# MMintLab/gelslim_depth

Measured on AMD Instinct MI355X. Metric: train frames/sec (320x427) at batch 32, higher is better.
Workload: dtype f32

## Files before the change

gelslim_depth_amd/csrc/gsd_convT.hip:

```cpp
#include "gsd_common.h"

namespace {

enum : int { CT_FWD = 1, CT_DGRAD = 2 };

struct ConvTParams {
  SrcD src;
  DstD dst;
  const float* wt;
  const float* bias;
  int K, M, Mpad, nchunks, mblocks;
  int N, H, W;
  int tiles_flat;
};

template <int MODE, int WM, int WN>
__global__ __launch_bounds__(256) void convT_kernel(const ConvTParams P) {
  constexpr int MT = 4, NT = 4;
  constexpr int BM = WM * 64, BN = WN * 64;
  constexpr int KSTEPS = 4;
  constexpr int WROWS = KSTEPS * 4;
  constexpr int WS = BM + 16;
  constexpr int PS = BN + 16;
  constexpr int W4 = WROWS * BM / 4;
// ... 171 lines not shown
      }
  }
}

struct ConvTFwdParams {
  SrcD src;
  DstD dst;
  const float* wt;
  const float* bias;
  int K, Kpad, M, nchunks, mblocks;
  int N, H, W, tiles_flat;
};

__device__ __attribute__((aligned(16))) const float gsd_zero16_ct[4] = {0.f, 0.f, 0.f, 0.f};

template <bool X4>
__global__ __launch_bounds__(256, 2) void convT_fwd_dma_kernel(const ConvTFwdParams P) {
  constexpr int BM = 128, BN = 128, KC = 32, MT = 4, NT = 4;
  constexpr int WIMG = KC * BM, XIMG = KC * BN, BUF = WIMG + XIMG;
  extern __shared__ __attribute__((aligned(16))) float smem[];
  const int tid = threadIdx.x, lane = tid & 63;
  const int wave = __builtin_amdgcn_readfirstlane(tid >> 6);
  const int wm = wave >> 1, wn = wave & 1;
  const int j = lane >> 4, l16 = lane & 15;

  const int lid = xcd_swizzle(blockIdx.x, gridDim.x);
  const int mb = lid % P.mblocks;
  const int pt = lid / P.mblocks;
  const int m0 = mb * BM;
  const long long q0 = (long long)pt * BN;
  const int HW = P.H * P.W;
  const long long QT = (long long)P.N * HW;

  float* sAff = smem + 2 * BUF;
  for (int c = tid; c < P.Kpad; c += 256) {
    float sc = 1.f, sh = 0.f;
    if (c < P.K && P.src.scale != nullptr) {
      sc = P.src.scale[c];
      sh = P.src.shift[c];
    }
    sAff[c] = sc;
    sAff[P.Kpad + c] = sh;
  }
  const float lo = P.src.relu ? 0.f : -__builtin_inff();

  const float* const wsrc = P.wt + (size_t)mb * P.Kpad * BM + lane * 4;
  const int xrow = X4 ? (lane >> 5) : 0;
  const int xpx = X4 ? (lane & 31) * 4 : lane;
  long long xo[X4 ? 1 : 2];
  bool xok[X4 ? 1 : 2];
#pragma unroll
  for (int i = 0; i < (X4 ? 1 : 2); ++i) {
    const long long q = q0 + xpx + 64 * i;
    xok[i] = q < QT;
    const int nn = xok[i] ? (int)(q / HW) : 0;
    xo[i] = (long long)nn * P.src.ns + (xok[i] ? (q - (long long)nn * HW) : 0);
  }
  auto fill = [&](int chunk, int buf) {
    float* Wb = smem + buf * BUF;
    float* Xb = Wb + WIMG;
    const float* wc = wsrc + (size_t)chunk * WIMG;
#pragma unroll
    for (int i = 0; i < 4; ++i) __builtin_amdgcn_global_load_lds(wc + (wave + 4 * i) * 256, Wb + (wave + 4 * i) * 256, 16, 0, 0);
    const int k0 = chunk * KC;
    if constexpr (X4) {
#pragma unroll
      for (int i = 0; i < 4; ++i) {
        const int r = 2 * (wave + 4 * i) + xrow;
        const float* g = (xok[0] && k0 + r < P.K) ? P.src.p + xo[0] + (long long)(k0 + r) * P.src.cs : &gsd_zero16_ct[0];
        __builtin_amdgcn_global_load_lds(g, Xb + (wave + 4 * i) * 256, 16, 0, 0);
      }
    } else {
#pragma unroll
      for (int i = 0; i < 16; ++i) {
        const int u = wave + 4 * i;
        const int r = u >> 1, hf = u & 1;
        const float* g = (xok[hf] && k0 + r < P.K) ? P.src.p + xo[hf] + (long long)(k0 + r) * P.src.cs : &gsd_zero16_ct[0];
        __builtin_amdgcn_global_load_lds(g, Xb + u * 64, 4, 0, 0);
      }
    }
  };

  f32x4 acc[MT][NT];
#pragma unroll
  for (int m = 0; m < MT; ++m)
#pragma unroll
    for (int t = 0; t < NT; ++t) acc[m][t] = f32x4{0.f, 0.f, 0.f, 0.f};

  const int a_off = j * BM + wm * 64 + l16 * 4;
  const int b_off = WIMG + j * BN + wn * 64 + l16 * 4;
  fill(0, 0);
  for (int chunk = 0; chunk < P.nchunks; ++chunk) {
    const int cur = chunk & 1;
    gsd_dma_barrier();
    if (chunk + 1 < P.nchunks) fill(chunk + 1, cur ^ 1);
    const float* Sb = smem + cur * BUF;
    const float* aff = sAff + chunk * KC + j;
    f32x4 av[2], bv[2];
    float sc[2], sh[2];
    av[0] = *reinterpret_cast<const f32x4*>(&Sb[a_off]);
    bv[0] = *reinterpret_cast<const f32x4*>(&Sb[b_off]);
    sc[0] = aff[0];
    sh[0] = aff[P.Kpad];
#pragma unroll
    for (int s = 0; s < KC / 4; ++s) {
      const int c = s & 1;
      if (s + 1 < KC / 4) {
        av[c ^ 1] = *reinterpret_cast<const f32x4*>(&Sb[a_off + (s + 1) * 4 * BM]);
        bv[c ^ 1] = *reinterpret_cast<const f32x4*>(&Sb[b_off + (s + 1) * 4 * BN]);
        sc[c ^ 1] = aff[(s + 1) * 4];
        sh[c ^ 1] = aff[P.Kpad + (s + 1) * 4];
      }
      float b[NT];
#pragma unroll
      for (int t = 0; t < NT; ++t) b[t] = fmaxf(fmaf(bv[c][t], sc[c], sh[c]), lo);
#pragma unroll
      for (int m = 0; m < MT; ++m)
#pragma unroll
        for (int t = 0; t < NT; ++t) acc[m][t] = mfma16(av[c][m], b[t], acc[m][t]);
    }
  }

  typedef float f32x4u __attribute__((ext_vector_type(4), aligned(4)));
  const DstD& D = P.dst;
  const long long qa = q0 + wn * 64 + l16 * 4;
  if (qa < QT) {
    const int na = (int)(qa / HW);
    const int pa = (int)(qa - (long long)na * HW);
    const int ha = pa / P.W, wa = pa - ha * P.W;
    const bool one_row = wa + 3 < P.W;
    if (one_row && qa + 3 < QT) {
      float* const o = D.p + (long long)na * D.ns + (long long)(2 * ha) * D.ws + 2 * wa;
#pragma unroll
      for (int m = 0; m < MT; ++m) {
        const int co = (m0 + wm * 64 + m * 16 + j * 4) >> 2;
        if (co < D.C) {
          const float bz = P.bias != nullptr ? P.bias[co] : 0.f;
          float* const oc = o + (long long)co * D.cs;
          *reinterpret_cast<f32x4u*>(oc) = f32x4{acc[m][0][0] + bz, acc[m][0][1] + bz, acc[m][1][0] + bz, acc[m][1][1] + bz};
          *reinterpret_cast<f32x4u*>(oc + 4) = f32x4{acc[m][2][0] + bz, acc[m][2][1] + bz, acc[m][3][0] + bz, acc[m][3][1] + bz};
          *reinterpret_cast<f32x4u*>(oc + D.ws) = f32x4{acc[m][0][2] + bz, acc[m][0][3] + bz, acc[m][1][2] + bz, acc[m][1][3] + bz};
          *reinterpret_cast<f32x4u*>(oc + D.ws + 4) = f32x4{acc[m][2][2] + bz, acc[m][2][3] + bz, acc[m][3][2] + bz, acc[m][3][3] + bz};
        }
      }
    } else {
#pragma unroll
      for (int t = 0; t < NT; ++t) {
        const long long q = qa + t;
        if (q >= QT) continue;
        const int nn = (int)(q / HW);
        const int p = (int)(q - (long long)nn * HW);
        const int h = p / P.W, w = p - h * P.W;
        float* const o = D.p + (long long)nn * D.ns + (long long)(2 * h) * D.ws + 2 * w;
#pragma unroll
        for (int m = 0; m < MT; ++m) {
          const int co = (m0 + wm * 64 + m * 16 + j * 4) >> 2;
          if (co < D.C) {
            const float bz = P.bias != nullptr ? P.bias[co] : 0.f;
            float* const oc = o + (long long)co * D.cs;
            *reinterpret_cast<float2*>(oc) = make_float2(acc[m][t][0] + bz, acc[m][t][1] + bz);
            *reinterpret_cast<float2*>(oc + D.ws) = make_float2(acc[m][t][2] + bz, acc[m][t][3] + bz);
          }
        }
      }
    }
  }
}

struct ConvTDgParams {
  SrcD src;
  DstD dst;
  const float* wt;
  int K, Kpad, M, nchunks, mblocks;
  int N, H, W, Wv, tiles_flat;
  const float* bw_raw;
  const float* bw_scale;
  const float* bw_shift;
  const float* bw_mean;
  const float* bw_invstd;
  float* partials;
  int Mpad;
};

template <bool BW>
__global__ __launch_bounds__(256, 2) void convT_dgrad_dma_kernel(const ConvTDgParams P) {
  constexpr int BM = 128, BN = 128, KC = 32, MT = 4, NT = 4;
  constexpr int WIMG = KC * BM, XIMG = (KC / 2) * (2 * BN), BUF = WIMG + XIMG;
  extern __shared__ __attribute__((aligned(16))) float smem[];
  const int tid = threadIdx.x, lane = tid & 63;
  const int wave = __builtin_amdgcn_readfirstlane(tid >> 6);
  const int wm = wave >> 1, wn = wave & 1;
  const int j = lane >> 4, l16 = lane & 15;

  const int lid = xcd_swizzle(blockIdx.x, gridDim.x);
  const int mb = lid % P.mblocks;
  const int pt = lid / P.mblocks;
  const int m0 = mb * BM;
  const long long q0 = (long long)pt * BN;
  const int HWv = P.H * P.Wv;
  const long long QT = (long long)P.N * HWv;

  const float* const wsrc = P.wt + (size_t)mb * P.Kpad * BM + lane * 4;
  const int pi = lane ^ ((lane >> 4) & 1);
  long long xo = 0;
  bool xok;
  {
    const long long q = q0 + 2 * pi;
    xok = q < QT;
    const int nn = xok ? (int)(q / HWv) : 0;
    const int rem = xok ? (int)(q - (long long)nn * HWv) : 0;
    const int h = rem / P.Wv, w = rem - h * P.Wv;
    xo = (long long)nn * P.src.ns + (long long)(2 * h) * P.src.ws + 2 * w;
  }
  auto fill = [&](int chunk, int buf) {
    float* Wb = smem + buf * BUF;
    float* Xb = Wb + WIMG;
    const float* wc = wsrc + (size_t)chunk * WIMG;
#pragma unroll
    for (int i = 0; i < 4; ++i) __builtin_amdgcn_global_load_lds(wc + (wave + 4 * i) * 256, Wb + (wave + 4 * i) * 256, 16, 0, 0);
#pragma unroll
    for (int i = 0; i < 4; ++i) {
      const int r = wave + 4 * i;
      const int co = chunk * 8 + (r >> 1);
      const float* g = (xok && co < P.src.C) ? P.src.p + xo + (long long)co * P.src.cs + (long long)(r & 1) * P.src.ws
                                              : &gsd_zero16_ct[0];
      __builtin_amdgcn_global_load_lds(g, Xb + r * 256, 16, 0, 0);
    }
  };

  f32x4 acc[MT][NT];
#pragma unroll
  for (int m = 0; m < MT; ++m)
#pragma unroll
    for (int t = 0; t < NT; ++t) acc[m][t] = f32x4{0.f, 0.f, 0.f, 0.f};

  const int a_off = (2 * j) * BM + wm * 64 + l16 * 4;
  const int lp = 2 * (wn * 16 + l16);
  const int b_off0 = WIMG + j * 256 + 4 * (lp ^ ((lp >> 4) & 1));
  const int b_off1 = WIMG + j * 256 + 4 * ((lp + 1) ^ (((lp + 1) >> 4) & 1));
  fill(0, 0);
  for (int chunk = 0; chunk < P.nchunks; ++chunk) {
    const int cur = chunk & 1;
    gsd_dma_barrier();
    if (chunk + 1 < P.nchunks) fill(chunk + 1, cur ^ 1);
    const float* Sb = smem + cur * BUF;
    f32x4 av[2], x0[2], x1[2];
    av[0] = *reinterpret_cast<const f32x4*>(&Sb[a_off]);
    x0[0] = *reinterpret_cast<const f32x4*>(&Sb[b_off0]);
    x1[0] = *reinterpret_cast<const f32x4*>(&Sb[b_off1]);
#pragma unroll
    for (int s = 0; s < KC / 4; ++s) {
      const int p = s >> 1, kw = s & 1, c = s & 1, pc = p & 1;
      if (s + 1 < KC / 4) {
        av[c ^ 1] = *reinterpret_cast<const f32x4*>(&Sb[a_off + ((s + 1) >> 1) * 8 * BM + ((s + 1) & 1) * BM]);
        if (kw == 1) {
          x0[pc ^ 1] = *reinterpret_cast<const f32x4*>(&Sb[b_off0 + (p + 1) * 4 * 256]);
          x1[pc ^ 1] = *reinterpret_cast<const f32x4*>(&Sb[b_off1 + (p + 1) * 4 * 256]);
        }
      }
      const float b[NT] = {x0[pc][kw], x0[pc][2 + kw], x1[pc][kw], x1[pc][2 + kw]};
#pragma unroll
      for (int m = 0; m < MT; ++m)
#pragma unroll
        for (int t = 0; t < NT; ++t) acc[m][t] = mfma16(av[c][m], b[t], acc[m][t]);
    }
  }

  typedef float f32x4u __attribute__((ext_vector_type(4), aligned(4)));
  const DstD& D = P.dst;
  const long long qa = q0 + wn * 64 + l16 * 4;
  if constexpr (BW) {
    __syncthreads();
    float* sBw = smem;
    if (tid < BM) {
      const int c = m0 + tid < D.C ? m0 + tid : 0;
      sBw[tid] = P.bw_scale[c];
      sBw[BM + tid] = P.bw_shift[c];
      sBw[2 * BM + tid] = P.bw_mean[c];
      sBw[3 * BM + tid] = P.bw_invstd[c];
    }
    __syncthreads();
    long long off[NT];
    bool ok[NT];
#pragma unroll
    for (int t = 0; t < NT; ++t) {
      const long long q = qa + t;
      ok[t] = q < QT;
      const int nn = ok[t] ? (int)(q / HWv) : 0;
      const int r = ok[t] ? (int)(q - (long long)nn * HWv) : 0;
      const int h = r / P.Wv, w = r - h * P.Wv;
      ok[t] = ok[t] && w < P.W;
      off[t] = (long long)nn * D.ns + (long long)h * D.ws + w;
    }
    const bool row4 = ok[0] && ok[3] && off[3] == off[0] + 3;
    float* const prow = P.partials + (size_t)(pt * 2 + wn) * (2 * P.Mpad);
#pragma unroll
    for (int m = 0; m < MT; ++m)
#pragma unroll
      for (int reg = 0; reg < 4; ++reg) {
        const int cl = wm * 64 + m * 16 + j * 4 + reg, ci = m0 + cl;
        const bool c_ok = ci < D.C;
        const long long cp = (long long)(c_ok ? ci : 0) * D.cs;
        const float bsc = sBw[cl], bsh = sBw[BM + cl], bmu = sBw[2 * BM + cl], bis = sBw[3 * BM + cl];
        float x[NT], dz[NT];
        if (row4) {
          const f32x4 tv = *reinterpret_cast<const f32x4u*>(P.bw_raw + cp + off[0]);
          x[0] = tv[0], x[1] = tv[1], x[2] = tv[2], x[3] = tv[3];
        } else {
#pragma unroll
          for (int t = 0; t < NT; ++t) x[t] = ok[t] ? P.bw_raw[cp + off[t]] : 0.f;
        }
        float s1 = 0.f, s2 = 0.f;
#pragma unroll
        for (int t = 0; t < NT; ++t) {
          dz[t] = (c_ok && ok[t] && fmaf(x[t], bsc, bsh) > 0.f) ? acc[m][t][reg] : 0.f;
          s1 += dz[t];
          s2 = fmaf(dz[t], (x[t] - bmu) * bis, s2);
        }
        if (c_ok) {
          if (row4) {
            *reinterpret_cast<f32x4u*>(D.p + cp + off[0]) = f32x4{dz[0], dz[1], dz[2], dz[3]};
          } else {
#pragma unroll
            for (int t = 0; t < NT; ++t)
              if (ok[t]) D.p[cp + off[t]] = dz[t];
          }
        }
        s1 = reduce16_to_lane15(s1);
        s2 = reduce16_to_lane15(s2);
        if (l16 == 15 && ci < P.Mpad) {
          prow[ci] = s1;
          prow[P.Mpad + ci] = s2;
        }
      }
    return;
  }
  if (qa < QT) {
    const int na = (int)(qa / HWv);
    const int ra = (int)(qa - (long long)na * HWv);
    const int ha = ra / P.Wv, wa = ra - ha * P.Wv;
    if (wa + 3 < P.W) {
      float* const o = D.p + (long long)na * D.ns + (long long)ha * D.ws + wa;
#pragma unroll
      for (int m = 0; m < MT; ++m)
#pragma unroll
        for (int reg = 0; reg < 4; ++reg) {
          const int ci = m0 + wm * 64 + m * 16 + j * 4 + reg;
          if (ci < D.C)
            *reinterpret_cast<f32x4u*>(o + (long long)ci * D.cs) = f32x4{acc[m][0][reg], acc[m][1][reg], acc[m][2][reg], acc[m][3][reg]};
// ... 6 lines not shown
        const int nn = (int)(q / HWv);
        const int r = (int)(q - (long long)nn * HWv);
        const int h = r / P.Wv, w = r - h * P.Wv;
        if (w >= P.W) continue;
        float* const o = D.p + (long long)nn * D.ns + (long long)h * D.ws + w;
#pragma unroll
        for (int m = 0; m < MT; ++m)
#pragma unroll
          for (int reg = 0; reg < 4; ++reg) {
            const int ci = m0 + wm * 64 + m * 16 + j * 4 + reg;
            if (ci < D.C) o[(long long)ci * D.cs] = acc[m][t][reg];
          }
      }
    }
  }
}

template <int MODE, int WM, int WN>
int launch(const ConvTParams& P, int grid, size_t lds, hipStream_t st, const char* what) {
  hipLaunchKernelGGL((convT_kernel<MODE, WM, WN>), dim3(grid), dim3(256), lds, st, P);
  GSD_LAUNCH_CHECK(what);
  return GSD_OK;
}

template <int MODE>
int run(ConvTParams& P, hipStream_t st, const char* what) {
  const bool wide = P.M <= 64;
  const int BM = wide ? 64 : 128, BN = wide ? 256 : 128;
  P.Mpad = round_up(P.M, 64);
  P.mblocks = ceil_div(P.M, BM);
// ... 26 lines not shown
  P.wt = wt;
  P.bias = bias;
  P.K = Cin;
  P.Kpad = round_up(Cin, 32);
  P.M = Cout * 4;
  P.nchunks = P.Kpad / 32;
  P.mblocks = ceil_div(P.M, 128);
  P.N = N; P.H = H; P.W = W;
  P.tiles_flat = (int)ceil_div64((int64_t)N * H * W, 128);
  const long grid = (long)P.tiles_flat * P.mblocks;
  GSD_REQUIRE(grid < 2147483647L, GSD_ERR_UNSUPPORTED, "gsd_convT2x2: grid too large");
  const size_t lds = (size_t)(2 * (32 * 128 + 32 * 128) + 2 * P.Kpad) * sizeof(float);
  GSD_REQUIRE(lds <= 80 * 1024, GSD_ERR_UNSUPPORTED, "gsd_convT2x2: Cin %d too large for the coefficient table", Cin);
  const bool x4 = gsd_env_int("GSD_CONVT_X4", 1) != 0 && ((uintptr_t)src->ptr & 15) == 0 && src->c_stride % 4 == 0 &&
                  src->n_stride % 4 == 0 && (H * W) % 4 == 0;
  if (x4) return gsd_launch<convT_fwd_dma_kernel<true>>("gsd_convT2x2", dim3((int)grid), dim3(256), lds, (hipStream_t)stream, P);
  return gsd_launch<convT_fwd_dma_kernel<false>>("gsd_convT2x2", dim3((int)grid), dim3(256), lds, (hipStream_t)stream, P);
}

extern "C" int gsd_convT2x2_dgrad_layout(const gsd_src* src, int Cin, int Cout, int N, int H, int W) {
  if (src == nullptr || Cin <= 0 || Cout <= 0 || N <= 0 || H <= 0 || W <= 0) return 3;
  if (gsd_env_int("GSD_CONVT_DG_DMA", 1) == 0) return 3;
  if ((W & 1) && src->slack < 2) return 3;
  if ((int64_t)N * src->n_stride >= (1LL << 40)) return 3;
  return 7;
}

extern "C" int gsd_convT2x2_dgrad(const gsd_src* src, const float* wt, int Cin, int Cout, const gsd_dst* dst, int N,
                                  int H, int W, void* stream) {
  return gsd_convT2x2_dgrad_as(gsd_convT2x2_dgrad_layout(src, Cin, Cout, N, H, W), src, wt, Cin, Cout, dst, N, H, W, stream);
}

// ... 24 lines not shown
    Q.wt = wt;
    Q.K = Cout * 4;
    Q.Kpad = round_up(Cout, 8) * 4;
    Q.M = Cin;
    Q.nchunks = Q.Kpad / 32;
    Q.mblocks = ceil_div(Cin, 128);
    Q.N = N; Q.H = H; Q.W = W;
    Q.Wv = round_up(W, 2);
    Q.tiles_flat = (int)ceil_div64((int64_t)N * H * Q.Wv, 128);
    const long grid = (long)Q.tiles_flat * Q.mblocks;
    GSD_REQUIRE(grid < 2147483647L, GSD_ERR_UNSUPPORTED, "gsd_convT2x2_dgrad: grid too large");
    const size_t lds = (size_t)(2 * (32 * 128 + 16 * 256)) * sizeof(float);
    Q.bw_raw = Q.bw_scale = Q.bw_shift = Q.bw_mean = Q.bw_invstd = nullptr;
    Q.partials = nullptr;
    Q.Mpad = 0;
    return gsd_launch<convT_dgrad_dma_kernel<false>>("gsd_convT2x2_dgrad", dim3((int)grid), dim3(256), lds, (hipStream_t)stream, Q);
  }
  ConvTParams P;
  P.src = to_srcd(*src);
  P.dst = to_dstd(*dst);
  P.wt = wt;
  P.bias = nullptr;
  P.K = Cout * 4;
  P.M = Cin;
  P.nchunks = ceil_div(Cout, 4);
  P.N = N; P.H = H; P.W = W;
  return run<CT_DGRAD>(P, (hipStream_t)stream, "gsd_convT2x2_dgrad");
}

static bool ct_dma_admits(const gsd_src* src, int Cin, int Cout, int N, int H, int W) {
  if (src == nullptr || Cin <= 0 || Cout <= 0 || N <= 0 || H <= 0 || W <= 0) return false;
// ... 29 lines not shown
  Q.wt = wt;
  Q.K = Cout * 4;
  Q.Kpad = round_up(Cout, 8) * 4;
  Q.M = Cin;
  Q.nchunks = Q.Kpad / 32;
  Q.mblocks = ceil_div(Cin, 128);
  Q.N = N; Q.H = H; Q.W = W;
  Q.Wv = round_up(W, 2);
  Q.tiles_flat = (int)ceil_div64((int64_t)N * H * Q.Wv, 128);
  Q.bw_raw = raw; Q.bw_scale = scale; Q.bw_shift = shift; Q.bw_mean = mean; Q.bw_invstd = invstd;
  Q.partials = partials;
  Q.Mpad = round_up(Cin, 64);
  const long grid = (long)Q.tiles_flat * Q.mblocks;
  GSD_REQUIRE(grid < 2147483647L, GSD_ERR_UNSUPPORTED, "gsd_convT2x2_dgrad_bnrelu: grid too large");
  const size_t lds = (size_t)(2 * (32 * 128 + 16 * 256)) * sizeof(float);
  return gsd_launch<convT_dgrad_dma_kernel<true>>("gsd_convT2x2_dgrad_bnrelu", dim3((int)grid), dim3(256), lds, (hipStream_t)stream, Q);
}
```

gelslim_depth_amd/csrc/gsd_wgrad.hip:

```cpp
#include "gsd_common.h"
#include "gsd_wgrad_internal.h"

#include <cstdlib>

struct WgradParams {
  SrcD a0, a1;
  SrcD dy;
  float* slabs;
  int M, Ncols, Cact;
  int N, H, W;
  int TH, TW, tiles_y, tiles_x, WR, WC, PS;
  int tiles_flat;
  int stages_total, splits, mblocks, nblocks;
};

template <int WM, int WN>
__global__ __launch_bounds__(256) void convT_wgrad_kernel(const WgradParams P) {
  constexpr int MT = 4, NTB = 4;
  constexpr int BMw = WM * 64, BNw = WN * 64;
  constexpr int DS = 66;

  extern __shared__ __attribute__((aligned(16))) float smem[];
  float* Al = smem;
  float* Xl = smem + BMw * DS;
// ... 391 lines not shown
#pragma unroll
      for (int m = 0; m < MT; ++m) a[m] = an[m];
#pragma unroll
      for (int t = 0; t < NTB; ++t) b[t] = fmaxf(fmaf(bn[t], sc[t], sh[t]), lo[t]);
      const int sn = s + 1 < 16 ? s + 1 : s;
#pragma unroll
      for (int m = 0; m < MT; ++m)
        an[m] = AX ? Al[a_off + m * 8 * 128 + 4 * ((2 * sn + (j >> 1)) ^ (l16 >> 1))] : Al[a_off + m * 16 * DS + 4 * sn];
#pragma unroll
      for (int t = 0; t < NTB; ++t) bn[t] = Bl[b_off + t * 16 * DSB + 4 * (BX ? (sn ^ l16) : sn)];
#pragma unroll
      for (int m = 0; m < MT; ++m)
#pragma unroll
        for (int t = 0; t < NTB; ++t) acc[m][t] = mfma16(a[m], b[t], acc[m][t]);
    }
  }
#pragma unroll
  for (int m = 0; m < MT; ++m)
#pragma unroll
    for (int reg = 0; reg < 4; ++reg) {
      const int mr = m0 + wm * 64 + m * 16 + j * 4 + reg;
      if (mr < P.M) {
#pragma unroll
        for (int t = 0; t < NTB; ++t) {
          const int col = n0 + wn * 64 + t * 16 + l16;
          if (col < P.Ncols) P.slabs[((size_t)split * P.M + mr) * P.Ncols + col] = acc[m][t][reg];
        }
      }
    }
}
// ... 287 lines not shown
  WgradParams P;
  P.a0 = to_srcd(*x);
  P.a1 = null_srcd();
  P.dy = to_srcd(*dy);
  P.slabs = workspace;
  P.M = M; P.Ncols = Cin; P.Cact = Cin;
  P.N = N; P.H = H; P.W = W;
  P.TH = P.TW = P.tiles_y = P.tiles_x = P.WR = P.WC = P.PS = 0;
  P.tiles_flat = pl.tiles_flat;
  P.stages_total = pl.stages_total; P.splits = pl.splits; P.mblocks = pl.mblocks; P.nblocks = pl.nblocks;
  const int grid = pl.splits * pl.mblocks * pl.nblocks;
  const size_t lds = (size_t)(pl.BMw * 66 + pl.BNw * 66) * sizeof(float);
  const bool bx = gsd_env_int("GSD_CONVT_WG_BX", 1) != 0 && (H * W) % 4 == 0 && ((uintptr_t)x->ptr & 15) == 0 &&
                  x->c_stride % 4 == 0 && x->n_stride % 4 == 0;
  const bool ax = bx && gsd_env_int("GSD_CONVT_WG_AX", 1) != 0;
  const char* const what = "gsd_convT2x2_wgrad";
  const hipStream_t st = (hipStream_t)stream;
  if (int e = pl.wide ? gsd_launch<convT_wgrad_kernel<1, 4>>(what, dim3(grid), dim3(256), lds, st, P)
              : ax    ? gsd_launch<convT_wgrad_dma_kernel<2>>(what, dim3(grid), dim3(256), lds, st, P)
              : bx    ? gsd_launch<convT_wgrad_dma_kernel<1>>(what, dim3(grid), dim3(256), lds, st, P)
                      : gsd_launch<convT_wgrad_dma_kernel<0>>(what, dim3(grid), dim3(256), lds, st, P))
    return e;
  launch_wgrad_reduce<1>(workspace, dw, pl.splits, M, Cin, (hipStream_t)stream);
  GSD_LAUNCH_CHECK("gsd_convT2x2_wgrad reduce");
  if (dbias != nullptr) {
    GSD_REQUIRE(dy->c_stride == (int64_t)4 * H * W && dy->n_stride == (int64_t)Cout * 4 * H * W, GSD_ERR_UNSUPPORTED,
                "gsd_convT2x2_wgrad: bias gradient needs a contiguous dy");
    float* ws2 = workspace + pl.slab_elems;
    hipLaunchKernelGGL(sum_planes_stage1, dim3(Cout, 64), dim3(256), 0, (hipStream_t)stream, dy->ptr, N, Cout,
                       (long long)4 * H * W, ws2);
    GSD_LAUNCH_CHECK("gsd_convT2x2_wgrad bias stage1");
    hipLaunchKernelGGL(sum_planes_stage2, dim3(ceil_div(Cout, 256)), dim3(256), 0, (hipStream_t)stream, ws2, Cout, 64,
                       dbias);
// ... 14 lines not shown
```

Baseline: 368.1.

## Interleave DMA prefetch with MFMA and add ring-buffered wgrad kernel for convT

Restructures the transposed-conv forward and dgrad DMA kernels so that the global-to-LDS loads for the next K chunk are issued piecewise between MFMA groups rather than in one burst. Steady-state chunks use 32-bit offset addressing without bounds checks, and only the tail chunk keeps the masked path. Bias and batchnorm parameters are loaded early, and sched_group_barrier hints interleave the affine+ReLU VALU work with MFMAs. A new ring-buffered wgrad kernel double-buffers half-stages and is selected when strides fit in 32-bit offsets. This adds code complexity and the risk that the compiler schedules the hinted regions poorly.

```diff
diff --git a/gelslim_depth_amd/csrc/gsd_convT.hip b/gelslim_depth_amd/csrc/gsd_convT.hip
--- a/gelslim_depth_amd/csrc/gsd_convT.hip
+++ b/gelslim_depth_amd/csrc/gsd_convT.hip
@@ -1,3 +1,5 @@
+#include <type_traits>
+
 #include "gsd_common.h"
 
 namespace {
@@ -209,10 +211,16 @@
 
 __device__ __attribute__((aligned(16))) const float gsd_zero16_ct[4] = {0.f, 0.f, 0.f, 0.f};
 
-template <bool X4>
+enum : int { CT_NEXT_NONE = 0, CT_NEXT_FULL = 1, CT_NEXT_TAIL = 2 };
+template <int V>
+using ct_const = std::integral_constant<int, V>;
+
+template <bool X4, bool O32>
 __global__ __launch_bounds__(256, 2) void convT_fwd_dma_kernel(const ConvTFwdParams P) {
   constexpr int BM = 128, BN = 128, KC = 32, MT = 4, NT = 4;
   constexpr int WIMG = KC * BM, XIMG = KC * BN, BUF = WIMG + XIMG;
+  constexpr int NH = X4 ? 1 : 2;
+  constexpr int NPX = X4 ? 4 : 16, NP = 4 + NPX;
   extern __shared__ __attribute__((aligned(16))) float smem[];
   const int tid = threadIdx.x, lane = tid & 63;
   const int wave = __builtin_amdgcn_readfirstlane(tid >> 6);
@@ -227,7 +235,119 @@
   const int HW = P.H * P.W;
   const long long QT = (long long)P.N * HW;
 
-  float* sAff = smem + 2 * BUF;
+  float* const sAff = smem + 2 * BUF;
+  const float lo = P.src.relu ? 0.f : -__builtin_inff();
+
+  const char* const wsrc = reinterpret_cast<const char*>(P.wt + (size_t)mb * P.Kpad * BM);
+  const unsigned wvo = lane * 16;
+  const int xrow = X4 ? (lane >> 5) : 0;
+  const int xpx = X4 ? (lane & 31) * 4 : lane;
+  const int n_first = (int)(q0 / HW);
+  long long xo[NH];
+  bool xok[NH];
+  unsigned xvo[NH];
+#pragma unroll
+  for (int i = 0; i < NH; ++i) {
+    const long long q = q0 + xpx + 64 * i;
+    xok[i] = q < QT;
+    const long long qc = xok[i] ? q : QT - (X4 ? 4 : 1);
+    const int nn = (int)(qc / HW);
+    const long long pix = qc - (long long)nn * HW;
+    xo[i] = xok[i] ? (long long)nn * P.src.ns + pix : 0;
+    xvo[i] = (unsigned)(((long long)(nn - n_first) * P.src.ns + pix + (long long)xrow * P.src.cs) * 4);
+  }
+  const float* const xbase = P.src.p + (long long)n_first * P.src.ns;
+  auto piece = [&](auto tail_c, const int pc, const int chunk, const int boff) {
+    constexpr bool TAIL = decltype(tail_c)::value;
+    float* Wb = smem + boff;
+    float* Xb = Wb + WIMG;
+    if (pc < 4) {
+      const int u = wave + 4 * pc;
+      __builtin_amdgcn_global_load_lds(reinterpret_cast<const float*>(wsrc + ((size_t)chunk * WIMG + u * 256) * sizeof(float) + wvo),
+                                       Wb + u * 256, 16, 0, 0);
+      return;
+    }
+    const int u = wave + 4 * (pc - 4);
+    const int k0 = chunk * KC;
+    const int rs = X4 ? 2 * u : (u >> 1), hf = X4 ? 0 : (u & 1);
+    const float* g;
+    if constexpr (O32 && !TAIL) {
+      g = reinterpret_cast<const float*>(reinterpret_cast<const char*>(xbase + (long long)(k0 + rs) * P.src.cs) + xvo[hf]);
+    } else {
+      const int r = rs + xrow;
+      const bool ok = TAIL ? (xok[hf] && k0 + r < P.K) : xok[hf];
+      g = ok ? P.src.p + xo[hf] + (long long)(k0 + r) * P.src.cs : &gsd_zero16_ct[0];
+    }
+    if constexpr (X4) __builtin_amdgcn_global_load_lds(g, Xb + u * 256, 16, 0, 0);
+    else __builtin_amdgcn_global_load_lds(g, Xb + u * 64, 4, 0, 0);
+  };
+
+  f32x4 acc[MT][NT];
+#pragma unroll
+  for (int m = 0; m < MT; ++m)
+#pragma unroll
+    for (int t = 0; t < NT; ++t) acc[m][t] = f32x4{0.f, 0.f, 0.f, 0.f};
+
+  const int a_off = j * BM + wm * 64 + l16 * 4;
+  const int b_off = WIMG + j * BN + wn * 64 + l16 * 4;
+  const bool ktail = (P.K % KC) != 0;
+
+  auto run_chunk = [&](auto next_c, const int chunk) {
+    constexpr int NEXT = decltype(next_c)::value;
+    const int ioff = (chunk & 1) * BUF;
+    gsd_dma_barrier();
+    const float* Sb = smem + ioff;
+    const float* aff = sAff + chunk * KC + j;
+    f32x4 av[2], bv;
+    float b[2][NT];
+    av[0] = *reinterpret_cast<const f32x4*>(&Sb[a_off]);
+    bv = *reinterpret_cast<const f32x4*>(&Sb[b_off]);
+    {
+      const float sc = aff[0], sh = aff[P.Kpad];
+#pragma unroll
+      for (int t = 0; t < NT; ++t) b[0][t] = fmaxf(fmaf(bv[t], sc, sh), lo);
+    }
+    __builtin_amdgcn_sched_barrier(0);
+#pragma unroll
+    for (int s = 0; s < KC / 4; ++s) {
+      const int c = s & 1;
+      const bool ahead = s + 1 < KC / 4;
+      float sc = 1.f, sh = 0.f;
+      if (ahead) {
+        av[c ^ 1] = *reinterpret_cast<const f32x4*>(&Sb[a_off + (s + 1) * 4 * BM]);
+        bv = *reinterpret_cast<const f32x4*>(&Sb[b_off + (s + 1) * 4 * BN]);
+        sc = aff[(s + 1) * 4];
+        sh = aff[P.Kpad + (s + 1) * 4];
+      }
+#pragma unroll
+      for (int m = 0; m < MT; ++m) {
+#pragma unroll
+        for (int t = 0; t < NT; ++t) acc[m][t] = mfma16(av[c][m], b[c][t], acc[m][t]);
+        if constexpr (NEXT != CT_NEXT_NONE) {
+          const int ord = s * MT + m;
+          if (ord < NP) piece(std::integral_constant<bool, NEXT == CT_NEXT_TAIL>{}, ord < NPX ? 4 + ord : ord - NPX, chunk + 1, BUF - ioff);
+        }
+        if (ahead && m >= 2) {
+#pragma unroll
+          for (int t = 2 * (m - 2); t < 2 * (m - 2) + 2; ++t) b[c ^ 1][t] = fmaxf(fmaf(bv[t], sc, sh), lo);
+#pragma unroll
+          for (int i = 0; i < 4; ++i) {
+            __builtin_amdgcn_sched_group_barrier(0x008, 1, 0);
+            __builtin_amdgcn_sched_group_barrier(0x002, 1, 0);
+          }
+        }
+        __builtin_amdgcn_sched_barrier(0);
+      }
+    }
+  };
+
+  if (ktail && P.nchunks == 1) {
+#pragma unroll
+    for (int pc = 0; pc < NP; ++pc) piece(std::true_type{}, pc, 0, 0);
+  } else {
+#pragma unroll
+    for (int pc = 0; pc < NP; ++pc) piece(std::false_type{}, pc, 0, 0);
+  }
   for (int c = tid; c < P.Kpad; c += 256) {
     float sc = 1.f, sh = 0.f;
     if (c < P.K && P.src.scale != nullptr) {
@@ -237,83 +357,18 @@
     sAff[c] = sc;
     sAff[P.Kpad + c] = sh;
   }
-  const float lo = P.src.relu ? 0.f : -__builtin_inff();
-
-  const float* const wsrc = P.wt + (size_t)mb * P.Kpad * BM + lane * 4;
-  const int xrow = X4 ? (lane >> 5) : 0;
-  const int xpx = X4 ? (lane & 31) * 4 : lane;
-  long long xo[X4 ? 1 : 2];
-  bool xok[X4 ? 1 : 2];
-#pragma unroll
-  for (int i = 0; i < (X4 ? 1 : 2); ++i) {
-    const long long q = q0 + xpx + 64 * i;
-    xok[i] = q < QT;
-    const int nn = xok[i] ? (int)(q / HW) : 0;
-    xo[i] = (long long)nn * P.src.ns + (xok[i] ? (q - (long long)nn * HW) : 0);
-  }
-  auto fill = [&](int chunk, int buf) {
-    float* Wb = smem + buf * BUF;
-    float* Xb = Wb + WIMG;
-    const float* wc = wsrc + (size_t)chunk * WIMG;
-#pragma unroll
-    for (int i = 0; i < 4; ++i) __builtin_amdgcn_global_load_lds(wc + (wave + 4 * i) * 256, Wb + (wave + 4 * i) * 256, 16, 0, 0);
-    const int k0 = chunk * KC;
-    if constexpr (X4) {
-#pragma unroll
-      for (int i = 0; i < 4; ++i) {
-        const int r = 2 * (wave + 4 * i) + xrow;
-        const float* g = (xok[0] && k0 + r < P.K) ? P.src.p + xo[0] + (long long)(k0 + r) * P.src.cs : &gsd_zero16_ct[0];
-        __builtin_amdgcn_global_load_lds(g, Xb + (wave + 4 * i) * 256, 16, 0, 0);
-      }
-    } else {
-#pragma unroll
-      for (int i = 0; i < 16; ++i) {
-        const int u = wave + 4 * i;
-        const int r = u >> 1, hf = u & 1;
-        const float* g = (xok[hf] && k0 + r < P.K) ? P.src.p + xo[hf] + (long long)(k0 + r) * P.src.cs : &gsd_zero16_ct[0];
-        __builtin_amdgcn_global_load_lds(g, Xb + u * 64, 4, 0, 0);
-      }
-    }
-  };
-
-  f32x4 acc[MT][NT];
-#pragma unroll
-  for (int m = 0; m < MT; ++m)
-#pragma unroll
-    for (int t = 0; t < NT; ++t) acc[m][t] = f32x4{0.f, 0.f, 0.f, 0.f};
-
-  const int a_off = j * BM + wm * 64 + l16 * 4;
-  const int b_off = WIMG + j * BN + wn * 64 + l16 * 4;
-  fill(0, 0);
-  for (int chunk = 0; chunk < P.nchunks; ++chunk) {
-    const int cur = chunk & 1;
-    gsd_dma_barrier();
-    if (chunk + 1 < P.nchunks) fill(chunk + 1, cur ^ 1);
-    const float* Sb = smem + cur * BUF;
-    const float* aff = sAff + chunk * KC + j;
-    f32x4 av[2], bv[2];
-    float sc[2], sh[2];
-    av[0] = *reinterpret_cast<const f32x4*>(&Sb[a_off]);
-    bv[0] = *reinterpret_cast<const f32x4*>(&Sb[b_off]);
-    sc[0] = aff[0];
-    sh[0] = aff[P.Kpad];
-#pragma unroll
-    for (int s = 0; s < KC / 4; ++s) {
-      const int c = s & 1;
-      if (s + 1 < KC / 4) {
-        av[c ^ 1] = *reinterpret_cast<const f32x4*>(&Sb[a_off + (s + 1) * 4 * BM]);
-        bv[c ^ 1] = *reinterpret_cast<const f32x4*>(&Sb[b_off + (s + 1) * 4 * BN]);
-        sc[c ^ 1] = aff[(s + 1) * 4];
-        sh[c ^ 1] = aff[P.Kpad + (s + 1) * 4];
-      }
-      float b[NT];
-#pragma unroll
-      for (int t = 0; t < NT; ++t) b[t] = fmaxf(fmaf(bv[c][t], sc[c], sh[c]), lo);
-#pragma unroll
-      for (int m = 0; m < MT; ++m)
-#pragma unroll
-        for (int t = 0; t < NT; ++t) acc[m][t] = mfma16(av[c][m], b[t], acc[m][t]);
-    }
+  float bz[MT];
+#pragma unroll
+  for (int m = 0; m < MT; ++m) {
+    const int co = (m0 + wm * 64 + m * 16 + j * 4) >> 2;
+    bz[m] = (P.bias != nullptr && co < P.dst.C) ? P.bias[co] : 0.f;
+  }
+  {
+    const int nfull = P.nchunks - 1 - (ktail && P.nchunks > 1 ? 1 : 0);
+    int chunk = 0;
+    for (; chunk < nfull; ++chunk) run_chunk(ct_const<CT_NEXT_FULL>{}, chunk);
+    if (chunk + 1 < P.nchunks) run_chunk(ct_const<CT_NEXT_TAIL>{}, chunk++);
+    run_chunk(ct_const<CT_NEXT_NONE>{}, chunk);
   }
 
   typedef float f32x4u __attribute__((ext_vector_type(4), aligned(4)));
@@ -330,12 +385,12 @@
       for (int m = 0; m < MT; ++m) {
         const int co = (m0 + wm * 64 + m * 16 + j * 4) >> 2;
         if (co < D.C) {
-          const float bz = P.bias != nullptr ? P.bias[co] : 0.f;
+          const float bm = bz[m];
           float* const oc = o + (long long)co * D.cs;
-          *reinterpret_cast<f32x4u*>(oc) = f32x4{acc[m][0][0] + bz, acc[m][0][1] + bz, acc[m][1][0] + bz, acc[m][1][1] + bz};
-          *reinterpret_cast<f32x4u*>(oc + 4) = f32x4{acc[m][2][0] + bz, acc[m][2][1] + bz, acc[m][3][0] + bz, acc[m][3][1] + bz};
-          *reinterpret_cast<f32x4u*>(oc + D.ws) = f32x4{acc[m][0][2] + bz, acc[m][0][3] + bz, acc[m][1][2] + bz, acc[m][1][3] + bz};
-          *reinterpret_cast<f32x4u*>(oc + D.ws + 4) = f32x4{acc[m][2][2] + bz, acc[m][2][3] + bz, acc[m][3][2] + bz, acc[m][3][3] + bz};
+          *reinterpret_cast<f32x4u*>(oc) = f32x4{acc[m][0][0] + bm, acc[m][0][1] + bm, acc[m][1][0] + bm, acc[m][1][1] + bm};
+          *reinterpret_cast<f32x4u*>(oc + 4) = f32x4{acc[m][2][0] + bm, acc[m][2][1] + bm, acc[m][3][0] + bm, acc[m][3][1] + bm};
+          *reinterpret_cast<f32x4u*>(oc + D.ws) = f32x4{acc[m][0][2] + bm, acc[m][0][3] + bm, acc[m][1][2] + bm, acc[m][1][3] + bm};
+          *reinterpret_cast<f32x4u*>(oc + D.ws + 4) = f32x4{acc[m][2][2] + bm, acc[m][2][3] + bm, acc[m][3][2] + bm, acc[m][3][3] + bm};
         }
       }
     } else {
@@ -351,10 +406,10 @@
         for (int m = 0; m < MT; ++m) {
           const int co = (m0 + wm * 64 + m * 16 + j * 4) >> 2;
           if (co < D.C) {
-            const float bz = P.bias != nullptr ? P.bias[co] : 0.f;
+            const float bm = bz[m];
             float* const oc = o + (long long)co * D.cs;
-            *reinterpret_cast<float2*>(oc) = make_float2(acc[m][t][0] + bz, acc[m][t][1] + bz);
-            *reinterpret_cast<float2*>(oc + D.ws) = make_float2(acc[m][t][2] + bz, acc[m][t][3] + bz);
+            *reinterpret_cast<float2*>(oc) = make_float2(acc[m][t][0] + bm, acc[m][t][1] + bm);
+            *reinterpret_cast<float2*>(oc + D.ws) = make_float2(acc[m][t][2] + bm, acc[m][t][3] + bm);
           }
         }
       }
@@ -377,7 +432,7 @@
   int Mpad;
 };
 
-template <bool BW>
+template <bool BW, bool O32>
 __global__ __launch_bounds__(256, 2) void convT_dgrad_dma_kernel(const ConvTDgParams P) {
   constexpr int BM = 128, BN = 128, KC = 32, MT = 4, NT = 4;
   constexpr int WIMG = KC * BM, XIMG = (KC / 2) * (2 * BN), BUF = WIMG + XIMG;
@@ -395,32 +450,46 @@
   const int HWv = P.H * P.Wv;
   const long long QT = (long long)P.N * HWv;
 
-  const float* const wsrc = P.wt + (size_t)mb * P.Kpad * BM + lane * 4;
+  const char* const wsrc = reinterpret_cast<const char*>(P.wt + (size_t)mb * P.Kpad * BM);
+  const unsigned wvo = lane * 16;
   const int pi = lane ^ ((lane >> 4) & 1);
+  const int n_first = (int)(q0 / HWv);
   long long xo = 0;
   bool xok;
+  unsigned xvo;
   {
     const long long q = q0 + 2 * pi;
     xok = q < QT;
-    const int nn = xok ? (int)(q / HWv) : 0;
-    const int rem = xok ? (int)(q - (long long)nn * HWv) : 0;
+    const long long qc = xok ? q : QT - 2;
+    const int nn = (int)(qc / HWv);
+    const int rem = (int)(qc - (long long)nn * HWv);
     const int h = rem / P.Wv, w = rem - h * P.Wv;
-    xo = (long long)nn * P.src.ns + (long long)(2 * h) * P.src.ws + 2 * w;
-  }
-  auto fill = [&](int chunk, int buf) {
-    float* Wb = smem + buf * BUF;
+    const long long po = (long long)(2 * h) * P.src.ws + 2 * w;
+    xo = xok ? (long long)nn * P.src.ns + po : 0;
+    xvo = (unsigned)(((long long)(nn - n_first) * P.src.ns + po) * 4);
+  }
+  const float* const xbase = P.src.p + (long long)n_first * P.src.ns;
+  auto piece = [&](auto tail_c, const int pc, const int chunk, const int boff) {
+    constexpr bool TAIL = decltype(tail_c)::value;
+    float* Wb = smem + boff;
     float* Xb = Wb + WIMG;
-    const float* wc = wsrc + (size_t)chunk * WIMG;
-#pragma unroll
-    for (int i = 0; i < 4; ++i) __builtin_amdgcn_global_load_lds(wc + (wave + 4 * i) * 256, Wb + (wave + 4 * i) * 256, 16, 0, 0);
-#pragma unroll
-    for (int i = 0; i < 4; ++i) {
-      const int r = wave + 4 * i;
-      const int co = chunk * 8 + (r >> 1);
-      const float* g = (xok && co < P.src.C) ? P.src.p + xo + (long long)co * P.src.cs + (long long)(r & 1) * P.src.ws
-                                              : &gsd_zero16_ct[0];
-      __builtin_amdgcn_global_load_lds(g, Xb + r * 256, 16, 0, 0);
-    }
+    if (pc < 4) {
+      const int u = wave + 4 * pc;
+      __builtin_amdgcn_global_load_lds(reinterpret_cast<const float*>(wsrc + ((size_t)chunk * WIMG + u * 256) * sizeof(float) + wvo),
+                                       Wb + u * 256, 16, 0, 0);
+      return;
+    }
+    const int r = wave + 4 * (pc - 4);
+    const int co = chunk * 8 + (r >> 1);
+    const long long ro = (long long)co * P.src.cs + (long long)(r & 1) * P.src.ws;
+    const float* g;
+    if constexpr (O32 && !TAIL) {
+      g = reinterpret_cast<const float*>(reinterpret_cast<const char*>(xbase + ro) + xvo);
+    } else {
+      const bool ok = TAIL ? (xok && co < P.src.C) : xok;
+      g = ok ? P.src.p + xo + ro : &gsd_zero16_ct[0];
+    }
+    __builtin_amdgcn_global_load_lds(g, Xb + r * 256, 16, 0, 0);
   };
 
   f32x4 acc[MT][NT];
@@ -433,16 +502,18 @@
   const int lp = 2 * (wn * 16 + l16);
   const int b_off0 = WIMG + j * 256 + 4 * (lp ^ ((lp >> 4) & 1));
   const int b_off1 = WIMG + j * 256 + 4 * ((lp + 1) ^ (((lp + 1) >> 4) & 1));
-  fill(0, 0);
-  for (int chunk = 0; chunk < P.nchunks; ++chunk) {
-    const int cur = chunk & 1;
+  const bool ktail = (P.src.C % 8) != 0;
+
+  auto run_chunk = [&](auto next_c, const int chunk) {
+    constexpr int NEXT = decltype(next_c)::value;
+    const int ioff = (chunk & 1) * BUF;
     gsd_dma_barrier();
-    if (chunk + 1 < P.nchunks) fill(chunk + 1, cur ^ 1);
-    const float* Sb = smem + cur * BUF;
+    const float* Sb = smem + ioff;
     f32x4 av[2], x0[2], x1[2];
     av[0] = *reinterpret_cast<const f32x4*>(&Sb[a_off]);
     x0[0] = *reinterpret_cast<const f32x4*>(&Sb[b_off0]);
     x1[0] = *reinterpret_cast<const f32x4*>(&Sb[b_off1]);
+    __builtin_amdgcn_sched_barrier(0);
 #pragma unroll
     for (int s = 0; s < KC / 4; ++s) {
       const int p = s >> 1, kw = s & 1, c = s & 1, pc = p & 1;
@@ -455,10 +526,41 @@
       }
       const float b[NT] = {x0[pc][kw], x0[pc][2 + kw], x1[pc][kw], x1[pc][2 + kw]};
 #pragma unroll
-      for (int m = 0; m < MT; ++m)
+      for (int m = 0; m < MT; ++m) {
 #pragma unroll
         for (int t = 0; t < NT; ++t) acc[m][t] = mfma16(av[c][m], b[t], acc[m][t]);
-    }
+        if constexpr (NEXT != CT_NEXT_NONE) {
+          const int ord = s * MT + m;
+          if (ord < 8) piece(std::integral_constant<bool, NEXT == CT_NEXT_TAIL>{}, ord < 4 ? 4 + ord : ord - 4, chunk + 1, BUF - ioff);
+        }
+        __builtin_amdgcn_sched_barrier(0);
+      }
+    }
+  };
+
+  if (ktail && P.nchunks == 1) {
+#pragma unroll
+    for (int pc = 0; pc < 8; ++pc) piece(std::true_type{}, pc, 0, 0);
+  } else {
+#pragma unroll
+    for (int pc = 0; pc < 8; ++pc) piece(std::false_type{}, pc, 0, 0);
+  }
+  float bwc[4] = {0.f, 0.f, 0.f, 0.f};
+  if constexpr (BW) {
+    if (tid < BM) {
+      const int c = m0 + tid < P.dst.C ? m0 + tid : 0;
+      bwc[0] = P.bw_scale[c];
+      bwc[1] = P.bw_shift[c];
+      bwc[2] = P.bw_mean[c];
+      bwc[3] = P.bw_invstd[c];
+    }
+  }
+  {
+    const int nfull = P.nchunks - 1 - (ktail && P.nchunks > 1 ? 1 : 0);
+    int chunk = 0;
+    for (; chunk < nfull; ++chunk) run_chunk(ct_const<CT_NEXT_FULL>{}, chunk);
+    if (chunk + 1 < P.nchunks) run_chunk(ct_const<CT_NEXT_TAIL>{}, chunk++);
+    run_chunk(ct_const<CT_NEXT_NONE>{}, chunk);
   }
 
   typedef float f32x4u __attribute__((ext_vector_type(4), aligned(4)));
@@ -468,11 +570,10 @@
     __syncthreads();
     float* sBw = smem;
     if (tid < BM) {
-      const int c = m0 + tid < D.C ? m0 + tid : 0;
-      sBw[tid] = P.bw_scale[c];
-      sBw[BM + tid] = P.bw_shift[c];
-      sBw[2 * BM + tid] = P.bw_mean[c];
-      sBw[3 * BM + tid] = P.bw_invstd[c];
+      sBw[tid] = bwc[0];
+      sBw[BM + tid] = bwc[1];
+      sBw[2 * BM + tid] = bwc[2];
+      sBw[3 * BM + tid] = bwc[3];
     }
     __syncthreads();
     long long off[NT];
@@ -489,22 +590,33 @@
     }
     const bool row4 = ok[0] && ok[3] && off[3] == off[0] + 3;
     float* const prow = P.partials + (size_t)(pt * 2 + wn) * (2 * P.Mpad);
-#pragma unroll
-    for (int m = 0; m < MT; ++m)
+    auto load_raw = [&](const int m, f32x4 (&xv)[4]) {
+#pragma unroll
+      for (int reg = 0; reg < 4; ++reg) {
+        const int ci = m0 + wm * 64 + m * 16 + j * 4 + reg;
+        const long long cp = (long long)(ci < D.C ? ci : 0) * D.cs;
+        if (row4) {
+          xv[reg] = *reinterpret_cast<const f32x4u*>(P.bw_raw + cp + off[0]);
+        } else {
+#pragma unroll
+          for (int t = 0; t < NT; ++t) xv[reg][t] = ok[t] ? P.bw_raw[cp + off[t]] : 0.f;
+        }
+      }
+    };
+    f32x4 xv[2][4];
+    load_raw(0, xv[0]);
+#pragma unroll
+    for (int m = 0; m < MT; ++m) {
+      if (m + 1 < MT) load_raw(m + 1, xv[(m + 1) & 1]);
 #pragma unroll
       for (int reg = 0; reg < 4; ++reg) {
         const int cl = wm * 64 + m * 16 + j * 4 + reg, ci = m0 + cl;
         const bool c_ok = ci < D.C;
         const long long cp = (long long)(c_ok ? ci : 0) * D.cs;
         const float bsc = sBw[cl], bsh = sBw[BM + cl], bmu = sBw[2 * BM + cl], bis = sBw[3 * BM + cl];
-        float x[NT], dz[NT];
-        if (row4) {
-          const f32x4 tv = *reinterpret_cast<const f32x4u*>(P.bw_raw + cp + off[0]);
-          x[0] = tv[0], x[1] = tv[1], x[2] = tv[2], x[3] = tv[3];
-        } else {
-#pragma unroll
-          for (int t = 0; t < NT; ++t) x[t] = ok[t] ? P.bw_raw[cp + off[t]] : 0.f;
-        }
+        const f32x4 tv = xv[m & 1][reg];
+        const float x[NT] = {tv[0], tv[1], tv[2], tv[3]};
+        float dz[NT];
         float s1 = 0.f, s2 = 0.f;
 #pragma unroll
         for (int t = 0; t < NT; ++t) {
@@ -528,6 +640,7 @@
           prow[P.Mpad + ci] = s2;
         }
       }
+    }
     return;
   }
   if (qa < QT) {
@@ -564,6 +677,12 @@
       }
     }
   }
+}
+
+bool ct_dg_o32(const gsd_src& src, int H, int Wv) {
+  const int64_t hwv = (int64_t)H * Wv;
+  return src.n_stride >= 0 && src.c_stride >= 0 && src.w_stride >= 0 &&
+         (127 / hwv + 1) * src.n_stride + (int64_t)(2 * H + 1) * src.w_stride + 4 < (1LL << 29);
 }
 
 template <int MODE, int WM, int WN>
@@ -620,8 +739,14 @@
   GSD_REQUIRE(lds <= 80 * 1024, GSD_ERR_UNSUPPORTED, "gsd_convT2x2: Cin %d too large for the coefficient table", Cin);
   const bool x4 = gsd_env_int("GSD_CONVT_X4", 1) != 0 && ((uintptr_t)src->ptr & 15) == 0 && src->c_stride % 4 == 0 &&
                   src->n_stride % 4 == 0 && (H * W) % 4 == 0;
-  if (x4) return gsd_launch<convT_fwd_dma_kernel<true>>("gsd_convT2x2", dim3((int)grid), dim3(256), lds, (hipStream_t)stream, P);
-  return gsd_launch<convT_fwd_dma_kernel<false>>("gsd_convT2x2", dim3((int)grid), dim3(256), lds, (hipStream_t)stream, P);
+  const int64_t hw = (int64_t)H * W;
+  const bool o32 = src->n_stride >= 0 && src->c_stride >= 0 && (127 / hw + 1) * src->n_stride + 32 * src->c_stride + hw < (1LL << 29);
+  const dim3 g((int)grid), b(256);
+  hipStream_t st = (hipStream_t)stream;
+  if (x4) return o32 ? gsd_launch<convT_fwd_dma_kernel<true, true>>("gsd_convT2x2", g, b, lds, st, P)
+                     : gsd_launch<convT_fwd_dma_kernel<true, false>>("gsd_convT2x2", g, b, lds, st, P);
+  return o32 ? gsd_launch<convT_fwd_dma_kernel<false, true>>("gsd_convT2x2", g, b, lds, st, P)
+             : gsd_launch<convT_fwd_dma_kernel<false, false>>("gsd_convT2x2", g, b, lds, st, P);
 }
 
 extern "C" int gsd_convT2x2_dgrad_layout(const gsd_src* src, int Cin, int Cout, int N, int H, int W) {
@@ -676,7 +801,9 @@
     Q.bw_raw = Q.bw_scale = Q.bw_shift = Q.bw_mean = Q.bw_invstd = nullptr;
     Q.partials = nullptr;
     Q.Mpad = 0;
-    return gsd_launch<convT_dgrad_dma_kernel<false>>("gsd_convT2x2_dgrad", dim3((int)grid), dim3(256), lds, (hipStream_t)stream, Q);
+    if (ct_dg_o32(*src, H, Q.Wv))
+      return gsd_launch<convT_dgrad_dma_kernel<false, true>>("gsd_convT2x2_dgrad", dim3((int)grid), dim3(256), lds, (hipStream_t)stream, Q);
+    return gsd_launch<convT_dgrad_dma_kernel<false, false>>("gsd_convT2x2_dgrad", dim3((int)grid), dim3(256), lds, (hipStream_t)stream, Q);
   }
   ConvTParams P;
   P.src = to_srcd(*src);
@@ -736,5 +863,7 @@
   const long grid = (long)Q.tiles_flat * Q.mblocks;
   GSD_REQUIRE(grid < 2147483647L, GSD_ERR_UNSUPPORTED, "gsd_convT2x2_dgrad_bnrelu: grid too large");
   const size_t lds = (size_t)(2 * (32 * 128 + 16 * 256)) * sizeof(float);
-  return gsd_launch<convT_dgrad_dma_kernel<true>>("gsd_convT2x2_dgrad_bnrelu", dim3((int)grid), dim3(256), lds, (hipStream_t)stream, Q);
-}
+  if (ct_dg_o32(*src, H, Q.Wv))
+    return gsd_launch<convT_dgrad_dma_kernel<true, true>>("gsd_convT2x2_dgrad_bnrelu", dim3((int)grid), dim3(256), lds, (hipStream_t)stream, Q);
+  return gsd_launch<convT_dgrad_dma_kernel<true, false>>("gsd_convT2x2_dgrad_bnrelu", dim3((int)grid), dim3(256), lds, (hipStream_t)stream, Q);
+}
diff --git a/gelslim_depth_amd/csrc/gsd_wgrad.hip b/gelslim_depth_amd/csrc/gsd_wgrad.hip
--- a/gelslim_depth_amd/csrc/gsd_wgrad.hip
+++ b/gelslim_depth_amd/csrc/gsd_wgrad.hip
@@ -2,6 +2,7 @@
 #include "gsd_wgrad_internal.h"
 
 #include <cstdlib>
+#include <type_traits>
 
 struct WgradParams {
   SrcD a0, a1;
@@ -429,6 +430,204 @@
 #pragma unroll
         for (int t = 0; t < NTB; ++t) acc[m][t] = mfma16(a[m], b[t], acc[m][t]);
     }
+  }
+#pragma unroll
+  for (int m = 0; m < MT; ++m)
+#pragma unroll
+    for (int reg = 0; reg < 4; ++reg) {
+      const int mr = m0 + wm * 64 + m * 16 + j * 4 + reg;
+      if (mr < P.M) {
+#pragma unroll
+        for (int t = 0; t < NTB; ++t) {
+          const int col = n0 + wn * 64 + t * 16 + l16;
+          if (col < P.Ncols) P.slabs[((size_t)split * P.M + mr) * P.Ncols + col] = acc[m][t][reg];
+        }
+      }
+    }
+}
+
+__global__ __launch_bounds__(256, 2) void convT_wgrad_ring_kernel(const WgradParams P) {
+  constexpr int MT = 4, NTB = 4, BMw = 128, BNw = 128;
+  constexpr int AIMG = 64 * 64, BIMG = 128 * 32, HALF = AIMG + BIMG;
+  extern __shared__ __attribute__((aligned(16))) float smem[];
+  const int tid = threadIdx.x, lane = tid & 63;
+  const int wave = __builtin_amdgcn_readfirstlane(tid >> 6);
+  const int wm = wave >> 1, wn = wave & 1;
+  const int j = lane >> 4, l16 = lane & 15;
+
+  const int lid = xcd_swizzle(blockIdx.x, gridDim.x);
+  const int per_split = P.mblocks * P.nblocks;
+  const int split = lid / per_split;
+  const int rem = lid - split * per_split;
+  const int mb = rem % P.mblocks, nb = rem / P.mblocks;
+  const int m0 = mb * BMw, n0 = nb * BNw;
+  const int s_begin = (int)((long long)split * P.stages_total / P.splits);
+  const int s_end = (int)((long long)(split + 1) * P.stages_total / P.splits);
+  const int HW = P.H * P.W;
+
+  float sc[NTB], sh[NTB], lo[NTB];
+#pragma unroll
+  for (int t = 0; t < NTB; ++t) {
+    const int c = n0 + wn * 64 + t * 16 + l16;
+    sc[t] = 1.f; sh[t] = 0.f; lo[t] = -__builtin_inff();
+    if (c < P.a0.C) {
+      if (P.a0.scale != nullptr) { sc[t] = P.a0.scale[c]; sh[t] = P.a0.shift[c]; }
+      if (P.a0.relu) lo[t] = 0.f;
+    }
+  }
+
+  f32x4 acc[MT][NTB];
+#pragma unroll
+  for (int m = 0; m < MT; ++m)
+#pragma unroll
+    for (int t = 0; t < NTB; ++t) acc[m][t] = f32x4{0.f, 0.f, 0.f, 0.f};
+
+  const int a_lr = lane >> 4, a_q = lane & 15;
+  const int a_sp = a_q ^ ((4 * wave + a_lr) & 7);
+  const int b_lr = lane >> 3, b_q = lane & 7;
+  const int b_sp = b_q ^ ((4 * wave + (b_lr >> 1)) & 7);
+  unsigned a_mok = 0, b_cok = 0;
+#pragma unroll
+  for (int i = 0; i < 4; ++i) {
+    a_mok |= (m0 + 2 * (4 * (wave + 4 * i) + a_lr) < P.M ? 1u : 0u) << i;
+    b_cok |= (n0 + 8 * (wave + 4 * i) + b_lr < P.a0.C ? 1u : 0u) << i;
+  }
+  const long long a_lane = (long long)(a_lr >> 1) * P.dy.cs + (long long)(a_lr & 1) * P.dy.W;
+  const unsigned b_lane = (unsigned)(((long long)b_lr * P.a0.cs + 4 * b_sp) * 4);
+  int f_n = s_begin / P.tiles_flat;
+  int f_tile = s_begin - f_n * P.tiles_flat;
+  int f_hs = 0;
+  const int d32h = 32 / P.W, d32w = 32 - d32h * P.W;
+  const int ha0 = (2 * a_sp) / P.W, wa0 = 2 * a_sp - ha0 * P.W;
+  int f_ha = (f_tile * 64 + 2 * a_sp) / P.W;
+  int f_wa = f_tile * 64 + 2 * a_sp - f_ha * P.W;
+  auto advance = [&]() {
+    f_hs ^= 1;
+    bool fresh = false;
+    if (f_hs == 0 && ++f_tile == P.tiles_flat) {
+      f_tile = 0;
+      ++f_n;
+      fresh = true;
+    }
+    if (fresh) {
+      f_ha = ha0;
+      f_wa = wa0;
+    } else {
+      f_ha += d32h;
+      f_wa += d32w;
+      if (f_wa >= P.W) {
+        f_wa -= P.W;
+        ++f_ha;
+      }
+    }
+  };
+  bool f_aok = false, f_bok = false, f_str = false;
+  unsigned f_avo = 0;
+  int f_pix0 = 0;
+  auto derive = [&]() {
+    f_pix0 = f_tile * 64 + f_hs * 32;
+    const int pa = f_pix0 + 2 * a_sp;
+    f_aok = pa < HW;
+    f_bok = f_pix0 + 4 * b_sp < HW;
+    f_str = f_aok && f_wa == P.W - 1;
+    f_avo = (unsigned)((a_lane + (long long)(2 * f_ha) * P.dy.W + 2 * f_wa) * 4);
+  };
+  auto a_src = [&](const int i) -> const float* {
+    const float* base = P.dy.p + (long long)f_n * P.dy.ns + (long long)((m0 >> 2) + 2 * (wave + 4 * i)) * P.dy.cs;
+    return reinterpret_cast<const float*>(reinterpret_cast<const char*>(base) + f_avo);
+  };
+  auto piece = [&](const int pc, float* img) {
+    if (pc < 4) {
+      const float* g = (f_aok && (a_mok >> pc & 1)) ? a_src(pc) : &gsd_zero16_wg[0];
+      __builtin_amdgcn_global_load_lds(g, img + (wave + 4 * pc) * 256, 16, 0, 0);
+    } else {
+      const int i = pc - 4;
+      const float* base = P.a0.p + (long long)f_n * P.a0.ns + (long long)(n0 + 8 * (wave + 4 * i)) * P.a0.cs + f_pix0;
+      const float* g = (f_bok && (b_cok >> i & 1)) ? reinterpret_cast<const float*>(reinterpret_cast<const char*>(base) + b_lane)
+                                                   : &gsd_zero16_wg[0];
+      __builtin_amdgcn_global_load_lds(g, img + AIMG + (wave + 4 * i) * 256, 16, 0, 0);
+    }
+  };
+  f32x2 a_fix[4];
+  bool fix_pend = false;
+  auto fix_loads = [&]() {
+    fix_pend = f_str;
+    if (__builtin_amdgcn_ballot_w64(f_str) != 0) {
+#pragma unroll
+      for (int i = 0; i < 4; ++i) {
+        a_fix[i] = f32x2{0.f, 0.f};
+        if (f_str && (a_mok >> i & 1)) a_fix[i] = *reinterpret_cast<const f32x2*>(a_src(i) + 2 * P.dy.W - 2 * f_wa);
+      }
+    }
+  };
+
+  const int a_rd = (wm * 32 + (l16 >> 1)) * 64 + 2 * (j & 1) + (l16 & 1);
+  const int a_y = (j >> 1) ^ (l16 >> 1);
+  const int b_rd = AIMG + (wn * 64 + l16) * 32 + j;
+  const int b_y = l16 >> 1;
+
+  auto run_half = [&](auto next_c, const int g) {
+    constexpr bool NEXT = decltype(next_c)::value;
+    float* const img = smem + (g & 1) * HALF;
+    float* const oimg = smem + ((g & 1) ^ 1) * HALF;
+    __builtin_amdgcn_s_waitcnt(0x0F70);
+    if (fix_pend) {
+#pragma unroll
+      for (int i = 0; i < 4; ++i) *reinterpret_cast<f32x2*>(&img[(wave + 4 * i) * 256 + lane * 4 + 2]) = a_fix[i];
+    }
+    __syncthreads();
+    if constexpr (NEXT) {
+      advance();
+      derive();
+      fix_loads();
+    }
+    float an[2][MT], braw[NTB], b[2][NTB];
+#pragma unroll
+    for (int m = 0; m < MT; ++m) an[0][m] = img[a_rd + m * 8 * 64 + 4 * a_y];
+#pragma unroll
+    for (int t = 0; t < NTB; ++t) braw[t] = img[b_rd + t * 16 * 32 + 4 * b_y];
+#pragma unroll
+    for (int t = 0; t < NTB; ++t) b[0][t] = fmaxf(fmaf(braw[t], sc[t], sh[t]), lo[t]);
+    __builtin_amdgcn_sched_barrier(0);
+#pragma unroll
+    for (int s = 0; s < 8; ++s) {
+      const int c = s & 1;
+      const bool ahead = s + 1 < 8;
+      if (ahead) {
+#pragma unroll
+        for (int m = 0; m < MT; ++m) an[c ^ 1][m] = img[a_rd + m * 8 * 64 + 4 * ((2 * (s + 1)) ^ a_y)];
+#pragma unroll
+        for (int t = 0; t < NTB; ++t) braw[t] = img[b_rd + t * 16 * 32 + 4 * ((s + 1) ^ b_y)];
+      }
+#pragma unroll
+      for (int m = 0; m < MT; ++m) {
+#pragma unroll
+        for (int t = 0; t < NTB; ++t) acc[m][t] = mfma16(an[c][m], b[c][t], acc[m][t]);
+        if constexpr (NEXT) {
+          if (s * MT + m < 8) piece(s * MT + m, oimg);
+        }
+        if (ahead && m >= 2) {
+#pragma unroll
+          for (int t = 2 * (m - 2); t < 2 * (m - 2) + 2; ++t) b[c ^ 1][t] = fmaxf(fmaf(braw[t], sc[t], sh[t]), lo[t]);
+#pragma unroll
+          for (int i = 0; i < 4; ++i) {
+            __builtin_amdgcn_sched_group_barrier(0x008, 1, 0);
+            __builtin_amdgcn_sched_group_barrier(0x002, 1, 0);
+          }
+        }
+        __builtin_amdgcn_sched_barrier(0);
+      }
+    }
+  };
+
+  const int G = 2 * (s_end - s_begin);
+  if (G > 0) {
+    derive();
+    fix_loads();
+#pragma unroll
+    for (int pc = 0; pc < 8; ++pc) piece(pc, smem);
+    for (int g = 0; g + 1 < G; ++g) run_half(std::true_type{}, g);
+    run_half(std::false_type{}, G - 1);
   }
 #pragma unroll
   for (int m = 0; m < MT; ++m)
@@ -746,9 +945,12 @@
   const bool bx = gsd_env_int("GSD_CONVT_WG_BX", 1) != 0 && (H * W) % 4 == 0 && ((uintptr_t)x->ptr & 15) == 0 &&
                   x->c_stride % 4 == 0 && x->n_stride % 4 == 0;
   const bool ax = bx && gsd_env_int("GSD_CONVT_WG_AX", 1) != 0;
+  const bool ring = ax && dy->c_stride >= 0 && x->c_stride >= 0 &&
+                    2 * dy->c_stride + (int64_t)(2 * H + 2) * dy->W + 4 < (1LL << 29) && 8 * x->c_stride + 64 < (1LL << 29);
   const char* const what = "gsd_convT2x2_wgrad";
   const hipStream_t st = (hipStream_t)stream;
   if (int e = pl.wide ? gsd_launch<convT_wgrad_kernel<1, 4>>(what, dim3(grid), dim3(256), lds, st, P)
+              : ring  ? gsd_launch<convT_wgrad_ring_kernel>(what, dim3(grid), dim3(256), lds, st, P)
               : ax    ? gsd_launch<convT_wgrad_dma_kernel<2>>(what, dim3(grid), dim3(256), lds, st, P)
               : bx    ? gsd_launch<convT_wgrad_dma_kernel<1>>(what, dim3(grid), dim3(256), lds, st, P)
                       : gsd_launch<convT_wgrad_dma_kernel<0>>(what, dim3(grid), dim3(256), lds, st, P))
```

Measured after the change: 370.4 (median of 6 runs). Within noise of the previous version (+0.6%).
